# eniac/Reef

Hardware: AMD Instinct MI355X
Metric: msm_scalar_point_pairs_per_sec (higher is better)
Workload: dtype u32

## Files before the change

### reef_amd/csrc/api.cpp

```cpp
#include <stdarg.h>
#include <stdio.h>
#include <string>
#include <vector>
#include <new>
#include <exception>
#include <stdlib.h>
#include <string.h>

#include <atomic>
#include <chrono>
#include <condition_variable>
#include <deque>
#include <memory>
#include <mutex>
#include <thread>
#include <type_traits>

#include "common.h"
#include "keccak.h"

namespace reef {

static thread_local char g_err[512] = "";

// ... 1056 lines not shown
        j.copy = nullptr;
        g_cache_bytes -= j.key->charged; g_host_bytes -= j.key->host_charged;
        j.key->charged = j.key->host_charged = 0;
        int expect = 1;
        j.key->state.compare_exchange_strong(expect, state, std::memory_order_release);
    }
    void execute(Job &j) {
        if (j.kind == RETIRE) {
            ReadyCtx victim = give(j.device, j.retire);
            victim.destroy();
            return;
        }
        if (j.kind == PURGE) {
            std::vector<ReadyCtx> gone;
            {
                std::lock_guard<std::mutex> lk(mu);
                for (auto &v : spares)
                    for (size_t i = 0; i < v.size();)
                        if (v[i].key && v[i].key->state.load() == 3) { gone.push_back(v[i]); v.erase(v.begin() + i); }
                        else ++i;
            }
            for (auto &r : gone) r.destroy();
            return;
        }
        DeviceGuard dg(j.device);
        if (!dg.ok) { if (j.kind == BUILD) fail_build(j, 4); return; }
        SharedKey &k = *j.key;
        if (k.n >= BG_STREAM_MIN_POINTS) (void)stream_pool().ensure_background_stream(k.device);
        reef_msm_opts o = {};
        o.bucket_groups = 1;
        o.byte_tables = 2;
        o.device = k.device;
        reef_msm_ctx *master = nullptr;
        if (reef_msm_ctx_create(&master, k.curve, (const reef_affine *)j.copy, k.n, REEF_HOST, &o) != REEF_OK) { fail_build(j, 4); return; }
        k.host_copy = j.copy;
        k.master = master;
        j.copy = nullptr;
        ReadyCtx spare;
        if (ready_ctx_make(&spare, j.key, k.n) != REEF_OK) spare.destroy();
        g_cache_builds += 1;
        ReadyCtx old;
        if (spare.ctx) {
            old = give(k.curve, spare);
            g_cache_spares += 1;
            if (old.ctx == spare.ctx) { spare.destroy(); old = ReadyCtx(); }
        }
        int expect = 1;
        if (!k.state.compare_exchange_strong(expect, 2, std::memory_order_release) && spare.ctx) {
            bool mine = false;
            {
                std::lock_guard<std::mutex> lk(mu);
                auto &v = spares[k.curve];
                for (size_t i = 0; i < v.size(); ++i)
                    if (v[i].ctx == spare.ctx) { v.erase(v.begin() + i); mine = true; break; }
            }
            if (mine) spare.destroy();
        }
        if (old.ctx) old.destroy();
    }
};
Builder &Builder::builder_instance() {
    static Builder *b = new Builder();
    return *b;
}
static Builder &builder() { return Builder::builder_instance(); }

void KeyTable::clear() {
// ... 305 lines not shown
```

### reef_amd/csrc/common.h

```cpp
#pragma once
#include <algorithm>
#include <atomic>
#include <mutex>
#include <optional>
#include <thread>
#include <stdio.h>
#include <stdlib.h>
#include <vector>
#include <hip/hip_runtime.h>
#include <stddef.h>
#include <stdint.h>

#include "../../include/reef_msm.h"

namespace reef {

void set_error(const char *fmt, ...) __attribute__((format(printf, 1, 2)));

#define REEF_HIP_TRY(expr)                                                                          \
    do {                                                                                            \
        hipError_t e_ = (expr);                                                                     \
        if (e_ != hipSuccess) {                                                                     \
            ::reef::set_error("%s: %s (%s:%d)", #expr, hipGetErrorString(e_), __FILE__, __LINE__);  \
            return e_ == hipErrorOutOfMemory ? REEF_ERR_OOM : REEF_ERR_HIP;                         \
        }                                                                                           \
    } while (0)

#define REEF_TRY(expr)                          \
    do {                                        \
        reef_status s_ = (expr);                \
        if (s_ != REEF_OK) return s_;           \
    } while (0)

inline const char *exp_env(const char *name) {
#ifdef REEF_EXPERIMENT
    return getenv(name);
#else
    (void)name;
    return nullptr;
#endif
}

struct DeviceGuard {
    int prev = -1;
    bool switched = false, ok = true;
    hipError_t err = hipSuccess;
    explicit DeviceGuard(int dev) {
        err = hipGetDevice(&prev);
        if (err == hipSuccess && prev != dev) {
            err = hipSetDevice(dev);
            switched = err == hipSuccess;
        }
        ok = err == hipSuccess;
        if (!ok) (void)hipGetLastError();
    }
    ~DeviceGuard() {
        if (switched) (void)hipSetDevice(prev);
    }
    DeviceGuard(const DeviceGuard &) = delete;
    DeviceGuard &operator=(const DeviceGuard &) = delete;
};
#define REEF_ON_DEVICE(dev)                                                                                   \
    ::reef::DeviceGuard dg_((dev));                                                                           \
    if (!dg_.ok) {                                                                                            \
        ::reef::set_error("cannot make device %d current: %s", (int)(dev), hipGetErrorString(dg_.err));       \
        return REEF_ERR_HIP;                                                                                  \
    }

inline std::atomic<uint64_t> g_devbuf_gen{0};
struct DevBuf {
    void *p = nullptr;
    size_t cap = 0;
    reef_status ensure(size_t bytes) {
        if (bytes <= cap) return REEF_OK;
// ... 469 lines not shown
```

### reef_amd/csrc/ec.h

```cpp
#pragma once
#include "field.h"

#if defined(__HIP_DEVICE_COMPILE__)
#define REEF_ANY(x) __any(x)
#else
#define REEF_ANY(x) (x)
#endif

namespace reef {

struct affine {
    fe x, y;
};
struct xyzz {
    fe x, y, zz, zzz;
};
struct alignas(16) affine256 {
    fe256 x, y;
};
struct alignas(16) jacobian256 {
    fe256 x, y, z;
};
struct alignas(16) xyzz_mem {
    u32 w[36];
// ... 35 lines not shown

template <int C> REEF_HD xyzz xyzz_dbl_affine(const affine &p) {
    xyzz r;
    const fe u = fe_dbl<C>(p.y);
    const fe v = fe_sqr<C>(u);
    const fe w = fe_mul<C>(u, v);
    const fe s = fe_mul<C>(p.x, v);
    const fe xx = fe_sqr<C>(p.x);
    const fe m = fe_add<C>(fe_dbl<C>(xx), xx);
    r.x = fe_sub<C, 4>(fe_sqr<C>(m), fe_dbl<C>(s));
    r.y = fe_sub<C, 2>(fe_mul<C>(m, fe_sub<C, 8>(s, r.x)),
                       fe_mul<C>(w, p.y));
    r.zz = v;
    r.zzz = w;
    return r;
}

template <int C> REEF_HD xyzz xyzz_dbl(const xyzz &p) {
    xyzz r;
    const fe u = fe_dbl<C>(p.y);
    const fe v = fe_sqr<C>(u);
    const fe w = fe_mul<C>(u, v);
    const fe s = fe_mul<C>(p.x, v);
    const fe xx = fe_sqr<C>(p.x);
    const fe m = fe_add<C>(fe_dbl<C>(xx), xx);
    r.x = fe_sub<C, 4>(fe_sqr<C>(m), fe_dbl<C>(s));
    r.y = fe_sub<C, 2>(fe_mul<C>(m, fe_sub<C, 8>(s, r.x)),
                       fe_mul<C>(w, p.y));
    r.zz = fe_mul<C>(v, p.zz);
    r.zzz = fe_mul<C>(w, p.zzz);
    return r;
}

template <int C> REEF_HD xyzz xyzz_madd_flag(const xyzz &a, bool a_known_empty, const affine &p) {
    const bool a_inf = a_known_empty || xyzz_is_inf<C>(a);
    const bool p_inf = affine_is_inf(p);
    const fe pp_ = fe_mul_sub<C, 8>(p.x, a.zz, a.x);
    const fe rr = fe_mul_sub<C, 4>(p.y, a.zzz, a.y);
    xyzz r;
    if (__builtin_expect(fe_is_zero<C>(pp_) && fe_is_zero<C>(rr) && !a_inf && !p_inf, 0)) {
        r = xyzz_dbl_affine<C>(p);
    } else {
        const fe pp = fe_sqr<C>(pp_);
        const fe ppp = fe_mul<C>(pp_, pp);
        const fe q = fe_mul<C>(a.x, pp);
        fe t;
#pragma unroll
        for (int i = 0; i < 9; ++i) t.l[i] = ppp.l[i] + 2u * q.l[i];
        REEF_SET_BOUND(t, REEF_GET_BOUND(ppp) + 2.0 * REEF_GET_BOUND(q));
        r.x = fe_sqr_sub<C, 4>(rr, t);
        r.y = fe_mul2_add<C>(rr, fe_sub<C, 8>(q, r.x), fe_neg<C, 4>(a.y), ppp);
        r.zz = fe_mul<C>(a.zz, pp);
        r.zzz = fe_mul<C>(a.zzz, ppp);
    }
    if (REEF_ANY(a_inf)) {
        xyzz from_p;
        from_p.x = p.x; from_p.y = p.y; from_p.zz = fe_one<C>(); from_p.zzz = from_p.zz;
        r = xyzz_select(a_inf, from_p, r);
    }
    if (REEF_ANY(p_inf)) r = xyzz_select(p_inf, a, r);
    return r;
}

template <int C> REEF_HD xyzz xyzz_madd(const xyzz &a, const affine &p) { return xyzz_madd_flag<C>(a, false, p); }

template <int C> REEF_HD xyzz xyzz_add(const xyzz &a, const xyzz &b) {
    const bool a_inf = xyzz_is_inf<C>(a);
    const bool b_inf = xyzz_is_inf<C>(b);
    const fe u1 = fe_mul<C>(a.x, b.zz);
    const fe u2 = fe_mul<C>(b.x, a.zz);
    const fe s1 = fe_mul<C>(a.y, b.zzz);
    const fe s2 = fe_mul<C>(b.y, a.zzz);
    const fe pp_ = fe_sub<C, 2>(u2, u1);
    const fe rr = fe_sub<C, 2>(s2, s1);
    xyzz r;
    if (__builtin_expect(fe_is_zero<C>(pp_) && fe_is_zero<C>(rr) && !a_inf && !b_inf, 0)) {
        r = xyzz_dbl<C>(a);
    } else {
        const fe pp = fe_sqr<C>(pp_);
        const fe ppp = fe_mul<C>(pp_, pp);
        const fe q = fe_mul<C>(u1, pp);
        const fe t = fe_add<C>(ppp, fe_dbl<C>(q));
        r.x = fe_sub<C, 4>(fe_sqr<C>(rr), t);
        r.y = fe_mul2_add<C>(rr, fe_sub<C, 8>(q, r.x), fe_neg<C, 2>(s1), ppp);
        r.zz = fe_mul<C>(fe_mul<C>(a.zz, b.zz), pp);
        r.zzz = fe_mul<C>(fe_mul<C>(a.zzz, b.zzz), ppp);
    }
    r = xyzz_select(a_inf, b, r);
    r = xyzz_select(b_inf, a, r);
    return r;
}

REEF_HD affine affine_from_table(const affine256 &m) {
    affine r;
    r.x = fe_from_table(m.x);
    r.y = fe_from_table(m.y);
    return r;
}
template <int C> REEF_HD affine256 affine_to_table(const affine &p) {
    affine256 m;
    m.x = fe_to_table<C>(p.x);
    m.y = fe_to_table<C>(p.y);
    return m;
}
template <int C> REEF_HD affine affine_from_abi(const affine256 &m) {
    affine r;
    r.x = fe_from_abi<C>(m.x);
    r.y = fe_from_abi<C>(m.y);
    return r;
}
template <int C> REEF_HD affine256 affine_to_abi(const affine &p) {
    affine256 m;
    m.x = fe_to_abi<C>(p.x);
    m.y = fe_to_abi<C>(p.y);
    return m;
}
REEF_HD xyzz xyzz_from_mem(const xyzz_mem &m) {
    xyzz r;
#pragma unroll
    for (int i = 0; i < 9; ++i) {
        r.x.l[i] = m.w[i]; r.y.l[i] = m.w[9 + i]; r.zz.l[i] = m.w[18 + i]; r.zzz.l[i] = m.w[27 + i];
    }
    REEF_SET_BOUND(r.x, 6.0); REEF_SET_BOUND(r.y, 3.6); REEF_SET_BOUND(r.zz, 1.6); REEF_SET_BOUND(r.zzz, 1.6);
    return r;
}
REEF_HD xyzz_mem xyzz_to_mem(const xyzz &p) {
    xyzz_mem m;
#if defined(REEF_BOUNDS)
    if (p.x.bound > 6.0 || p.y.bound > 3.6 || p.zz.bound > 1.6 || p.zzz.bound > 1.6) REEF_BOUND_FAIL("xyzz_to_mem: invariant");
#endif
#pragma unroll
// ... 62 lines not shown
```

### reef_amd/csrc/engine.inc

```
#include <algorithm>
#include <atomic>
#include <mutex>
#include <string.h>
#include <vector>

#include "common.h"
#include "glv_host.h"
#include "host_combine.h"

namespace reef {

static_assert(sizeof(fe256) == sizeof(reef_fe), "fe256 layout");
static_assert(sizeof(affine256) == sizeof(reef_affine), "affine256 layout");
static_assert(sizeof(jacobian256) == sizeof(reef_jacobian), "jacobian256 layout");
static_assert(sizeof(xyzz_mem) == 144, "xyzz_mem layout");

static constexpr u32 MAX_LDS_KEYS = 32768;
static constexpr u32 MAX_SCAN_KEYS = SCAN_TILE * 1024;
static constexpr u32 SORT_SHIFT = 8;
static constexpr u64 TWO_LEVEL_MIN_ENTRIES = 1u << 20;
static constexpr u32 DEFAULT_L0 = 0;

static inline u32 ceil_div(u64 a, u64 b) { return (u32)((a + b - 1) / b); }
static inline u64 round_up(u64 a, u64 b) { return (a + b - 1) / b * b; }
static inline u32 windows_for(u32 c) { return (256 + c - 1) / c; }

static u32 choose_window(size_t n, u32 groups_mode ) {
    if (groups_mode == 1) {
        return n < 61440 ? 13u : n < 180224 ? 15u : 17u;
    }
    u32 best_c = 4;
    double best = 1e300;
    for (u32 c = 3; c <= 20; ++c) {
        const u32 W = windows_for(c);
        const u32 G = groups_mode == 0 ? W : std::min(groups_mode, W);
        const double nb = (double)(1u << (c - 1));
        const double digits = (double)(255 / c) + ((255 % c) == 0 ? 0.5 : 1.0);
        const double cost = digits * (double)n + (G == 1 ? 10.0 : 4.0) * G * nb;
        if (cost < best) { best = cost; best_c = c; }
    }
    return best_c;
}

template <int C> struct Key {
    affine256 *tables = nullptr;
    size_t n = 0, cap = 0;
    u32 c = 0, W = 0, G = 0, T = 0;
    affine256 *small_tab = nullptr;
    size_t small_n = 0;
    affine256 *wide_tab = nullptr;
    std::atomic<size_t> wide_n{0};
    std::atomic<int> wide_state{0};
    hipStream_t wide_stream = nullptr;
    hipEvent_t wide_event = nullptr;
    void *wide_stage = nullptr;
    int *wide_abort = nullptr;
    std::mutex wide_mu;
    std::atomic<int> refs{1};
    int device = 0;
};

template <int C> struct Ctx {
    Key<C> *key = nullptr;
    hipStream_t stream = nullptr;
    StreamLease lease;
    std::mutex mu;
    u32 opt_c = 0, opt_G = 0, L0 = DEFAULT_L0, opt_tables = 0;
    DevBuf scalars, blinds, hpoint, result, tmp_xyzz, maxbits;
    DevBuf dig, counts, tile_sums, bstart, entries;
    DevBuf bstart1, seg_first, seg_counts, entries1;
    DevBuf bucket_acc, lkeys[2], lvals[2];
    DevBuf rowcol, group_sums;
    static constexpr int EV_RING = 32;
    hipEvent_t evr[EV_RING][4] = {};
    bool ev_pending[EV_RING] = {};
    int ev_next = 0, ev_last = -1;
    hipEvent_t *ev = nullptr;
    double sum_total_ms = 0, sum_accum_ms = 0;
    u64 timed_calls = 0;
    jacobian256 *pinned = nullptr;
// ... 47 lines not shown
    REEF_HIP_TRY(hipEventSynchronize(ctx->evr[slot][3]));
    float t = 0, a = 0;
    REEF_HIP_TRY(hipEventElapsedTime(&t, ctx->evr[slot][0], ctx->evr[slot][3]));
    REEF_HIP_TRY(hipEventElapsedTime(&a, ctx->evr[slot][1], ctx->evr[slot][2]));
    ctx->sum_total_ms += t;
    ctx->sum_accum_ms += a;
    ctx->timed_calls += 1;
    ctx->ev_pending[slot] = false;
    return REEF_OK;
}
template <int C> static reef_status ctx_begin_timing(Ctx<C> *ctx) {
    const int slot = ctx->ev_next;
    REEF_TRY(ctx_harvest<C>(ctx, slot));
    ctx->ev = ctx->evr[slot];
    ctx->ev_last = slot;
    ctx->ev_next = (slot + 1) % Ctx<C>::EV_RING;
    return REEF_OK;
}

template <int C> static void wide_drop(Key<C> *k) {
    if (k->wide_abort) *(volatile int *)k->wide_abort = 1;
    if (k->wide_stream) (void)hipStreamSynchronize(k->wide_stream);
    if (k->wide_event) { (void)hipEventDestroy(k->wide_event); k->wide_event = nullptr; }
    if (k->wide_stream) { (void)hipStreamDestroy(k->wide_stream); k->wide_stream = nullptr; }
    if (k->wide_stage) { (void)hipFree(k->wide_stage); k->wide_stage = nullptr; }
    if (k->wide_tab) { (void)hipFree(k->wide_tab); k->wide_tab = nullptr; }
    if (k->wide_abort) { (void)hipHostFree(k->wide_abort); k->wide_abort = nullptr; }
    k->wide_n.store(0);
    k->wide_state.store(0);
}
template <int C> static void key_release(Key<C> *k) {
    if (k && --k->refs == 0) {
        if (k->tables) (void)hipFree(k->tables);
        if (k->small_tab) (void)hipFree(k->small_tab);
        wide_drop(k);
        delete k;
    }
}

static reef_status set_lds_limit(const void *fn) {
    REEF_HIP_TRY(hipFuncSetAttribute(fn, hipFuncAttributeMaxDynamicSharedMemorySize, (int)(MAX_LDS_KEYS * sizeof(u32))));
    return REEF_OK;
}

static reef_status engine_init_once() {
    static std::once_flag once;
    static reef_status st = REEF_OK;
    std::call_once(once, [] {
        auto f = []() -> reef_status {
            REEF_TRY(set_lds_limit((const void *)k_count));
            REEF_TRY(set_lds_limit((const void *)k_recode_count<REEF_CURVE>));
            REEF_TRY(set_lds_limit((const void *)k_scatter<false>));
            REEF_TRY(set_lds_limit((const void *)k_scatter<true>));
            REEF_TRY(set_lds_limit((const void *)k_row_count));
            REEF_TRY(set_lds_limit((const void *)k_row_scatter));
            return REEF_OK;
        };
        st = f();
    });
    return st;
}

static reef_status plan_for(size_t n, uint32_t c_opt, uint32_t g_opt, uint32_t *c, uint32_t *w, uint32_t *g, uint32_t *t);

static inline size_t small_table_points(size_t n) { return (size_t)SMALL_WINDOWS * SMALL_DIGITS * n; }
template <int C> static reef_status small_build(Ctx<C> *ctx, const affine256 *pts, size_t n, affine256 *out) {
// ... 167 lines not shown
    hipStream_t st = ctx->stream;
    const u64 total = (u64)WIDE_WINDOWS * n;
    const u32 per = wide_per(total);
    const u32 wgs = (u32)ceil_div(total, (u64)256 * per);
    REEF_TRY(ctx->wide_dig.ensure(total * sizeof(short)));
    const u32 lvl2 = ceil_div(wgs, 64);
    REEF_TRY(ctx->wide_partial.ensure(((size_t)wgs + lvl2) * sizeof(xyzz_mem)));
    xyzz_mem *p1 = ctx->wide_partial.template as<xyzz_mem>(), *p2 = p1 + wgs;
    if (ctx->timing) {
        REEF_TRY(ctx_begin_timing<C>(ctx));
        REEF_HIP_TRY(hipEventRecord(ctx->ev[0], st));
    }
    hipLaunchKernelGGL(k_wide_recode<C>, dim3(ceil_div(n, 256)), dim3(256), 0, st, d_scalars, (u32)n, (int)is_mont, ctx->wide_dig.template as<short>());
    if (ctx->timing) REEF_HIP_TRY(hipEventRecord(ctx->ev[1], st));
    hipLaunchKernelGGL((k_wide_accum<C, false>), dim3(wgs), dim3(256), 0, st, (const affine256 *)key->wide_tab, (u32)key->wide_n.load(),
                       (const short *)ctx->wide_dig.template as<short>(), (u32)n, per, 0u, p1);
    if (ctx->timing) REEF_HIP_TRY(hipEventRecord(ctx->ev[2], st));
    const xyzz_mem *last = p1;
    u32 cnt = wgs;
    if (cnt > 512) {
        hipLaunchKernelGGL(k_wide_reduce<C>, dim3(lvl2), dim3(256), 0, st, (const xyzz_mem *)p1, cnt, p2);
        last = p2;
        cnt = lvl2;
    }
    hipLaunchKernelGGL(k_small_final<C>, dim3(1), dim3(256), 0, st, last, cnt, d_out);
    if (ctx->timing) {
        REEF_HIP_TRY(hipEventRecord(ctx->ev[3], st));
        ctx->ev_pending[ctx->ev_last] = true;
    }
    REEF_HIP_TRY(hipGetLastError());
    return REEF_OK;
}

template <int C>
static reef_status key_build(Ctx<C> *ctx, const reef_affine *bases, size_t n, int loc) {
    Key<C> *key = ctx->key;
    u32 c, W, G, T;
    REEF_TRY(plan_for(n, ctx->opt_c, ctx->opt_G, &c, &W, &G, &T));
    wide_drop(key);
    const size_t need = (size_t)T * std::max<size_t>(n, 1);
    if (need > key->cap) {
        if (key->tables) { (void)hipFree(key->tables); key->tables = nullptr; key->cap = 0; }
        REEF_HIP_TRY(hipMalloc((void **)&key->tables, need * sizeof(affine256)));
        key->cap = need;
    }
    key->n = n; key->c = c; key->W = W; key->G = G; key->T = T;
    ctx->sym_bits = ctx->symw_bits = 0;
    graphs_clear(ctx);
    if (n == 0) return REEF_OK;
    const affine256 *src = (const affine256 *)bases;
    const u32 per_batch = T > 1 ? (u32)std::max<size_t>(1, std::min<size_t>(T - 1, (size_t(1) << 30) / (n * sizeof(xyzz_mem)))) : 1;
    size_t staging_bytes = T > 1 ? (size_t)per_batch * n * sizeof(xyzz_mem) : 0;
    if (G == 1 && n <= SMALL_N_MAX) staging_bytes = std::max(staging_bytes, (small_table_points(n) + (size_t)SMALL_WINDOWS * n) * sizeof(xyzz_mem));
    if (loc != REEF_DEVICE) staging_bytes = std::max(staging_bytes, n * sizeof(affine256));
    REEF_TRY(ctx->tmp_xyzz.ensure(std::max<size_t>(staging_bytes, 16)));
    if (loc != REEF_DEVICE) {
        REEF_HIP_TRY(hipMemcpyAsync(ctx->tmp_xyzz.p, bases, n * sizeof(affine256), hipMemcpyHostToDevice, ctx->stream));
        src = ctx->tmp_xyzz.template as<affine256>();
    }
    hipLaunchKernelGGL(k_import_key<C>, dim3(ceil_div(n, 256)), dim3(256), 0, ctx->stream, src, (u32)n, key->tables);
    if (T > 1) {
        for (u32 j = 1; j < T; j += per_batch) {
            const u32 cnt = std::min(per_batch, T - j);
            hipLaunchKernelGGL(k_shift_chain<C>, dim3(ceil_div(n, 64)), dim3(64), 0, ctx->stream, key->tables + (size_t)(j - 1) * n, (u32)n, c * G, cnt, 0,
                               ctx->tmp_xyzz.template as<xyzz_mem>());
            hipLaunchKernelGGL((k_xyzz_normalize<C, false>), dim3(ceil_div(ceil_div((size_t)cnt * n, NORM_PER), 256)), dim3(256), 0, ctx->stream,
                               ctx->tmp_xyzz.template as<xyzz_mem>(), (u32)((size_t)cnt * n), key->tables + (size_t)j * n);
        }
    }
    key->small_n = 0;
    if (G == 1 && n <= SMALL_N_MAX) {
        if (key->small_tab) { (void)hipFree(key->small_tab); key->small_tab = nullptr; }
        REEF_HIP_TRY(hipMalloc((void **)&key->small_tab, small_table_points(n) * sizeof(affine256)));
        REEF_TRY(small_build<C>(ctx, key->tables, n, key->small_tab));
        key->small_n = n;
    }
    REEF_HIP_TRY(hipGetLastError());
    REEF_HIP_TRY(hipStreamSynchronize(ctx->stream));
    if (ctx->tmp_xyzz.cap > (size_t(96) << 20)) ctx->tmp_xyzz.release();
    if (wide_start<C>(key, ctx->opt_tables) != REEF_OK) {
        (void)hipGetLastError();
        wide_drop(key);
    }
    if (ctx->opt_tables == 1) wide_poll<C>(key, true);
    return REEF_OK;
}

template <int C> static void ctx_free(Ctx<C> *ctx) {
    if (!ctx) return;
    ctx_free(ctx->side);
    ctx_free(ctx->side_batch);
    for (auto &e : ctx->batch_ev)
        if (e) (void)hipEventDestroy(e);
    graphs_clear(ctx);
    for (DevBuf *b : {&ctx->scalars, &ctx->blinds, &ctx->hpoint, &ctx->dig, &ctx->counts, &ctx->bstart, &ctx->bstart1, &ctx->seg_first,
                      &ctx->seg_counts, &ctx->entries1, &ctx->sym_table, &ctx->sym_tmp, &ctx->sym_u8, &ctx->tile_sums,
                      &ctx->entries, &ctx->bucket_acc, &ctx->rowcol, &ctx->group_sums, &ctx->result,
                      &ctx->tmp_xyzz, &ctx->maxbits, &ctx->wsum, &ctx->deep_dig, &ctx->deep_part, &ctx->h_tab, &ctx->small_partial, &ctx->wide_dig, &ctx->wide_partial, &ctx->lkeys[0], &ctx->lkeys[1], &ctx->lvals[0], &ctx->lvals[1]})
        b->release();
    for (auto &q : ctx->evr)
        for (auto &e : q)
            if (e) (void)hipEventDestroy(e);
// ... 389 lines not shown
            hipLaunchKernelGGL(k_seg_plan, dim3(1), dim3(1024), 0, st, bstart_c, NBTc, seg_first);
            hipLaunchKernelGGL(k_fine_count<true>, dim3(nseg_max), dim3(1024), fine * sizeof(u32), st, (const void *)e1, bstart_c, seg_first, NBTc, shift, seg_counts);
            hipLaunchKernelGGL(k_fine_offsets, dim3(NBTc), dim3(fine), 0, st, bstart_c, seg_first, NBTc, shift, seg_counts, bstart);
            if (word_entries)
                hipLaunchKernelGGL((k_fine_scatter<true, true>), dim3(nseg_max), dim3(1024), fine * sizeof(u32), st, (const void *)e1, bstart_c, seg_first, NBTc, shift, seg_counts,
                                   (void *)ctx->entries.template as<u32x2>());
            else
                hipLaunchKernelGGL((k_fine_scatter<true, false>), dim3(nseg_max), dim3(1024), fine * sizeof(u32), st, (const void *)e1, bstart_c, seg_first, NBTc, shift, seg_counts,
                                   (void *)ctx->entries.template as<u32x2>());
        } else {
            hipLaunchKernelGGL(k_scatter<false>, dim3(S, groups_total, NBc / sh.KB), dim3(1024), sh.KB * sizeof(u32), st, dig, sh, ctx->counts.template as<u32>(), (void *)e1);
            hipLaunchKernelGGL(k_seg_plan, dim3(1), dim3(1024), 0, st, bstart_c, NBTc, seg_first);
            hipLaunchKernelGGL(k_fine_count<false>, dim3(nseg_max), dim3(1024), fine * sizeof(u32), st, (const void *)e1, bstart_c, seg_first, NBTc, shift, seg_counts);
            hipLaunchKernelGGL(k_fine_offsets, dim3(NBTc), dim3(fine), 0, st, bstart_c, seg_first, NBTc, shift, seg_counts, bstart);
            hipLaunchKernelGGL((k_fine_scatter<false, false>), dim3(nseg_max), dim3(1024), fine * sizeof(u32), st, (const void *)e1, bstart_c, seg_first, NBTc, shift, seg_counts,
                               (void *)ctx->entries.template as<u32x2>());
        }
    } else if (!row_mode) {
        hipLaunchKernelGGL(k_scatter<false>, dim3(S, groups_total, NB / sh.KB), dim3(1024), sh.KB * sizeof(u32), st, dig, sh, ctx->counts.template as<u32>(),
                           (void *)ctx->entries.template as<u32x2>());
    } else {
        hipLaunchKernelGGL(k_row_scatter, dim3(ceil_div(pl.rows, rsh.rows_per_block)), dim3(1024),
                           rsh.rows_per_block * pl.G * NB * sizeof(u32), st, dig, rsh, bstart, ctx->entries.template as<u32x2>());
    }

    if (ctx->timing) REEF_HIP_TRY(hipEventRecord(ctx->ev[1], st));
    const bool fused = merge_is_fused<C>(ctx, nchunks0);
    {
        const dim3 ag(ceil_div(nchunks0, 256)), ab(256);
        const void *ent = (const void *)ctx->entries.template as<u32x2>();
        xyzz_mem *bacc = ctx->bucket_acc.template as<xyzz_mem>();
        u32 *ok = ctx->lkeys[fused ? 1 : 0].template as<u32>();
        xyzz_mem *ov = ctx->lvals[fused ? 1 : 0].template as<xyzz_mem>();
        if (fused && word_entries) hipLaunchKernelGGL((k_accum0<C, true, true>), ag, ab, 0, st, ctx->key->tables, ent, bstart + NBT, L0, nchunks0, bacc, ok, ov, NBT);
        else if (fused) hipLaunchKernelGGL((k_accum0<C, true, false>), ag, ab, 0, st, ctx->key->tables, ent, bstart + NBT, L0, nchunks0, bacc, ok, ov, 0u);
        else if (word_entries) hipLaunchKernelGGL((k_accum0<C, false, true>), ag, ab, 0, st, ctx->key->tables, ent, bstart + NBT, L0, nchunks0, bacc, ok, ov, NBT);
        else hipLaunchKernelGGL((k_accum0<C, false, false>), ag, ab, 0, st, ctx->key->tables, ent, bstart + NBT, L0, nchunks0, bacc, ok, ov, 0u);
    }
    if (ctx->timing) REEF_HIP_TRY(hipEventRecord(ctx->ev[2], st));
    launch_partial_merge<C>(ctx, nchunks0, ctx->bucket_acc.template as<xyzz_mem>(), fused);

    const u32 lg = pl.c - 1;
    const u32 c2 = (lg + 1) / 2, c1 = lg - c2;
    const u32 per_group = (1u << c1) + (1u << c2);
    const u32 rc_waves = groups_total * per_group;
    xyzz_mem *gsum = ctx->group_sums.template as<xyzz_mem>();
    if (group_sums_out && ctx->pinned && (size_t)groups_total * sizeof(xyzz_mem) <= Ctx<C>::PINNED_POINTS * sizeof(jacobian256))
        gsum = (xyzz_mem *)ctx->pinned;
    const bool direct = !group_sums_out && pl.G == 1;
    static const int skip_reduce = [] { const char *e = exp_env("REEF_MSM_SKIP_REDUCE"); return e ? atoi(e) : 0; }();
    const int lanes = rowcol >= 0 ? rowcol : rowcol_lanes<C>(ctx, NB);
    auto launch_rowcol = [&](auto lps) {
        constexpr int LPS = decltype(lps)::value;
        hipLaunchKernelGGL((k_reduce_rowcol<C, LPS>), dim3(ceil_div(ceil_div(rc_waves, 64u / LPS), 4)), dim3(256), 0, st, ctx->bucket_acc.template as<xyzz_mem>(),
                           bstart, c1, c2, groups_total, ctx->rowcol.template as<xyzz_mem>());
    };
    if (skip_reduce == 1) {
        if (group_sums_out) *group_sums_out = gsum;
    } else if (ctx->coop) {
        REEF_TRY(ctx->wsum.ensure((u64)groups_total * 4 * sizeof(xyzz_mem)));
        ++ctx->rowcol_calls[lanes != 0];
        if (skip_reduce == 2) {}
        else if (lanes == 16) launch_rowcol(std::integral_constant<int, 16>{});
        else if (lanes == 32) launch_rowcol(std::integral_constant<int, 32>{});
        else if (lanes == 64) launch_rowcol(std::integral_constant<int, 64>{});
        else
        hipLaunchKernelGGL(k_reduce_rowcol_coop<C>, dim3(rc_waves), dim3(256), 0, st, ctx->bucket_acc.template as<xyzz_mem>(), bstart, c1, c2,
                           groups_total, ctx->rowcol.template as<xyzz_mem>());
        hipLaunchKernelGGL(k_reduce_weighted_coop<C>, dim3(groups_total, 2), dim3(256), 0, st, ctx->rowcol.template as<xyzz_mem>(), c1, c2,
                           ctx->wsum.template as<xyzz_mem>());
// ... 1201 lines not shown
```

### reef_amd/csrc/msm_kernels.inc

```
#include "ec.h"
#include "ec_coop.h"
#include "glv_consts.h"

namespace reef {

static constexpr u32 KEY_INVALID = 0xffffffffu;
static constexpr int WAVE = 64;

template <int C> struct Kern;

__device__ __forceinline__ void latency_critical() { __builtin_amdgcn_s_setprio(3); }

__device__ __forceinline__ u32 extract_bits(const fe256 &k, u32 off, u32 c) {
    const u32 limb = off >> 5, sh = off & 31u;
    u32 lo = 0, hi = 0;
#pragma unroll
    for (u32 l = 0; l < 8; ++l) {
        lo = (l == limb) ? k.w[l] : lo;
        hi = (l == limb + 1) ? k.w[l] : hi;
    }
    u64 v = (((u64)hi << 32) | lo) >> sh;
    return (u32)v & ((1u << c) - 1u);
}

__device__ __forceinline__ fe256 load_fe256(const fe256 *p) {
    const u32x4 *q = reinterpret_cast<const u32x4 *>(p);
    const u32x4 a = q[0], b = q[1];
    fe256 d;
    d.w[0] = a.x; d.w[1] = a.y; d.w[2] = a.z; d.w[3] = a.w;
    d.w[4] = b.x; d.w[5] = b.y; d.w[6] = b.z; d.w[7] = b.w;
    return d;
}
__device__ __forceinline__ void store_fe256(fe256 *p, const fe256 &s) {
    u32x4 *q = reinterpret_cast<u32x4 *>(p);
    q[0] = mk_u32x4(s.w[0], s.w[1], s.w[2], s.w[3]);
    q[1] = mk_u32x4(s.w[4], s.w[5], s.w[6], s.w[7]);
}
__device__ __forceinline__ affine256 load_affine256(const affine256 *p) {
    affine256 r;
    r.x = load_fe256(&p->x);
    r.y = load_fe256(&p->y);
    return r;
}
__device__ __forceinline__ void store_affine256(affine256 *p, const affine256 &s) {
    store_fe256(&p->x, s.x);
    store_fe256(&p->y, s.y);
}
__device__ __forceinline__ jacobian256 load_jacobian256(const jacobian256 *p) {
    jacobian256 r;
    r.x = load_fe256(&p->x); r.y = load_fe256(&p->y); r.z = load_fe256(&p->z);
    return r;
}
__device__ __forceinline__ void store_jacobian256(jacobian256 *p, const jacobian256 &s) {
    store_fe256(&p->x, s.x); store_fe256(&p->y, s.y); store_fe256(&p->z, s.z);
}
__device__ __forceinline__ affine load_table_point(const affine256 *p) { return affine_from_table(load_affine256(p)); }
__device__ __forceinline__ xyzz load_xyzz(const xyzz_mem *p) {
    const u32x4 *q = reinterpret_cast<const u32x4 *>(p);
    xyzz_mem m;
#pragma unroll
    for (int i = 0; i < 9; ++i) {
        const u32x4 v = q[i];
        m.w[4 * i] = v.x; m.w[4 * i + 1] = v.y; m.w[4 * i + 2] = v.z; m.w[4 * i + 3] = v.w;
    }
    return xyzz_from_mem(m);
}
__device__ __forceinline__ xyzz load_xyzz_coop(const xyzz_mem *p) {
    const u32x4 *q = reinterpret_cast<const u32x4 *>(p);
    xyzz_mem m;
#pragma unroll
    for (int i = 0; i < 9; ++i) {
        const u32x4 v = q[i];
        m.w[4 * i] = coop_launder(v.x); m.w[4 * i + 1] = coop_launder(v.y); m.w[4 * i + 2] = coop_launder(v.z); m.w[4 * i + 3] = coop_launder(v.w);
    }
    return xyzz_from_mem(m);
}
__device__ __forceinline__ void store_xyzz(xyzz_mem *p, const xyzz &s) {
    const xyzz_mem m = xyzz_to_mem(s);
    u32x4 *q = reinterpret_cast<u32x4 *>(p);
#pragma unroll
    for (int i = 0; i < 9; ++i) q[i] = mk_u32x4(m.w[4 * i], m.w[4 * i + 1], m.w[4 * i + 2], m.w[4 * i + 3]);
}
__device__ __forceinline__ xyzz shfl_xyzz(const xyzz &a, int src_lane) {
    xyzz_mem m = xyzz_to_mem(a);
#pragma unroll
    for (int i = 0; i < 36; ++i) m.w[i] = __shfl(m.w[i], src_lane, WAVE);
    return xyzz_from_mem(m);
}

// ... 447 lines not shown
    for (u32 k = threadIdx.x; k < nkeys; k += blockDim.x) cur[k] = bucket_start[key0 + k];
    __syncthreads();
    const size_t n = (size_t)sh.rows * sh.row_len;
    const u32 cnt = nrows * sh.row_len;
    for (u32 w = 0; w < sh.W; ++w) {
        const u32 *d = dig + (size_t)w * n + (size_t)r0 * sh.row_len;
        const u32 g = w % sh.G, j = w / sh.G;
        for (u32 e = threadIdx.x; e < cnt; e += blockDim.x) {
            const u32 v = d[e];
            const u32 mag = v & 0x7fffffffu;
            if (mag) {
                const u32 row = e / sh.row_len, col = e - row * sh.row_len;
                const u32 rel = (row * sh.G + g) * sh.NB + mag - 1u;
                const u32 pos = atomicAdd(&cur[rel], 1u);
                entries[pos] = mk_u32x2(key0 + rel, (j * sh.n_ctx + col) | (v & 0x80000000u));
            }
        }
    }
}

template <int C, bool COOP>
__device__ __forceinline__ void merge_wave(u32 ka, u32 kb, xyzz v, xyzz bv, u32 wave_id, int lane, int role, CoopLds *L,
                                           xyzz_mem *__restrict__ bucket_acc, u32 *__restrict__ out_keys, xyzz_mem *__restrict__ out_vals);


__device__ __forceinline__ u32 bucket_of(const u32 *__restrict__ bs, u32 nbt, u32 p) {
    u32 lo = 0, hi = nbt;
    while (hi - lo > 1) {
        const u32 mid = (lo + hi) >> 1;
        if (bs[mid] <= p) lo = mid; else hi = mid;
    }
    return lo;
}
template <int C, bool FUSED, bool WORD = false>
__global__ void __launch_bounds__(256) k_accum0(const affine256 *__restrict__ tables, const void *__restrict__ entries_,
                                               const u32 *__restrict__ m_ptr, u32 L0,
                                               u32 nchunks, xyzz_mem *__restrict__ bucket_acc, u32 *__restrict__ out_keys,
                                               xyzz_mem *__restrict__ out_vals, u32 nbt = 0) {
    __shared__ xyzz_mem stash[FUSED ? 256 : 1];
    const u32 t = blockIdx.x * blockDim.x + threadIdx.x;
    if constexpr (FUSED) {
        if (((t >> 6) << 6) >= nchunks) return;
    } else {
        if (t >= nchunks) return;
    }
    const u32 M = *m_ptr;
    while (L0 > 8 && (u64)(L0 >> 1) * nchunks >= M) L0 >>= 1;
    const u32 start = t * L0;
    u32 key_a = KEY_INVALID, key_b = KEY_INVALID;
    xyzz tail = xyzz_identity();
    if (t < nchunks && start < M) {
        const u32 end = min(start + L0, M);
        const u32 cnt = end - start;
        const u32x2 *mine = static_cast<const u32x2 *>(entries_) + start;
        const u32 *mine1 = static_cast<const u32 *>(entries_) + start;
        const u32 *bs = m_ptr - nbt;
        u32 cur_key, pay, boundary = 0;
        bool lo_open, ro_open = false;
        u32 prev_key = KEY_INVALID, next_key = KEY_INVALID;
        if constexpr (WORD) {
            cur_key = bucket_of(bs, nbt, start);
            boundary = bs[cur_key + 1];
            lo_open = bs[cur_key] < start;
            pay = mine1[0];
        } else {
            prev_key = start > 0 ? static_cast<const u32x2 *>(entries_)[start - 1].x : KEY_INVALID;
            next_key = end < M ? static_cast<const u32x2 *>(entries_)[end].x : KEY_INVALID;
            const u32x2 e0 = mine[0];
            cur_key = e0.x;
            pay = e0.y;
            lo_open = prev_key == cur_key;
        }
        affine256 raw = load_affine256(tables + (pay & 0x7fffffffu));
        xyzz acc = xyzz_identity();
        bool acc_empty = true;
        bool first_run = true;
        for (u32 k = 0; k < cnt; ++k) {
            u32 nkey = cur_key, npay = 0;
            affine256 nraw = raw;
            if (k + 1 < cnt) {
                if constexpr (WORD) {
                    npay = mine1[k + 1];
                    if (start + k + 1 == boundary) {
                        nkey = cur_key + 1;
                        if (bs[nkey + 1] == boundary) nkey = bucket_of(bs, nbt, boundary);
                    }
                } else {
                    const u32x2 e = mine[k + 1];
                    nkey = e.x;
                    npay = e.y;
                }
                nraw = load_affine256(tables + (npay & 0x7fffffffu));
            }
            affine pt = affine_from_table(raw);
            pt.y = fe_select((pay >> 31) != 0 && !affine_is_inf(pt), fe_neg<C, 2>(pt.y), pt.y);
            acc = xyzz_madd_flag<C>(acc, acc_empty, pt);
            acc_empty = false;
            const bool last = (k + 1 == cnt);
            if (last || nkey != cur_key) {
                const bool lo = first_run && lo_open;
                bool ro;
                if constexpr (WORD) ro = last && boundary > end;
                else ro = last && next_key == cur_key;
                if (!lo && !ro) {
                    store_xyzz(bucket_acc + cur_key, acc);
                } else if (lo) {
                    if constexpr (FUSED) store_xyzz(&stash[threadIdx.x], acc);
                    else store_xyzz(out_vals + 2 * (size_t)t, acc);
                    key_a = cur_key;
                    if (ro) {
                        if constexpr (!FUSED) store_xyzz(out_vals + 2 * (size_t)t + 1, xyzz_identity());
                        key_b = cur_key;
                    }
                } else {
                    if constexpr (FUSED) tail = acc;
                    else store_xyzz(out_vals + 2 * (size_t)t + 1, acc);
                    key_b = cur_key;
                }
                first_run = false;
                acc = xyzz_identity();
                acc_empty = true;
                if constexpr (WORD) { if (!last) boundary = bs[nkey + 1]; }
            }
            cur_key = nkey; pay = npay; raw = nraw;
        }
        (void)ro_open; (void)prev_key;
    }
    if constexpr (FUSED) {
        latency_critical();
// ... 904 lines not shown
    __shared__ BatchInvShared inv_sh;
    const u32 t = blockIdx.x * blockDim.x + threadIdx.x;
    const u64 i0 = (u64)t * NORM_PER;
    fe zp[NORM_PER], pre[NORM_PER];
    fe acc = fe_one<C>();
#pragma unroll
    for (int k = 0; k < NORM_PER; ++k) {
        zp[k] = fe_one<C>();
        if (i0 + k < n) {
            const xyzz p = load_xyzz(in + i0 + k);
            const fe prod = fe_mul<C>(p.zz, p.zzz);
            zp[k] = fe_select(fe_is_zero<C>(prod), zp[k], prod);
        }
        pre[k] = acc;
        acc = fe_mul<C>(acc, zp[k]);
    }
    fe inv = block_batch_inverse<C>(acc, inv_sh);
#pragma unroll
    for (int k = NORM_PER - 1; k >= 0; --k) {
        const fe ti = fe_mul<C>(inv, pre[k]);
        inv = fe_mul<C>(inv, zp[k]);
        if (i0 + k < n) {
            const affine a = xyzz_to_affine_with_inv<C>(load_xyzz(in + i0 + k), ti);
            store_affine256(out + i0 + k, ABI_OUT ? affine_to_abi<C>(a) : affine_to_table<C>(a));
        }
    }
}

template <int C>
__global__ void __launch_bounds__(256) k_import_key(const affine256 *__restrict__ src, u32 n, affine256 *__restrict__ dst) {
    const u32 i = blockIdx.x * blockDim.x + threadIdx.x;
    if (i >= n) return;
    store_affine256(dst + i, affine_to_table<C>(affine_from_abi<C>(load_affine256(src + i))));
}

template <int C>
__global__ void __launch_bounds__(64) k_shift_chain(const affine256 *__restrict__ src, u32 n, u32 shift, u32 count, int first,
                                                    xyzz_mem *__restrict__ tmp) {
    const u32 i = blockIdx.x * blockDim.x + threadIdx.x;
    if (i >= n) return;
    xyzz p = xyzz_from_affine<C>(load_table_point(src + i));
    for (u32 j = 0; j < count; ++j) {
        if (!(first && j == 0))
            for (u32 s = 0; s < shift; ++s) p = xyzz_dbl<C>(p);
        store_xyzz(tmp + (size_t)j * n + i, p);
    }
}


template <int C>
__global__ void __launch_bounds__(256) k_sym_multiples(const affine256 *__restrict__ gens, u32 n, u32 lb, u32 hb, xyzz_mem *__restrict__ lo_out,
                                                      xyzz_mem *__restrict__ hi_out) {
    const u32 t = blockIdx.x * blockDim.x + threadIdx.x;
    const u32 j = t >> 1, part = t & 1u;
    if (j >= n || (part == 1 && hb == 0)) return;
    const affine g = load_table_point(gens + j);
    const u32 count = 1u << (part ? hb : lb);
    xyzz_mem *out = (part ? hi_out : lo_out) + (size_t)j * count;
    xyzz step = xyzz_from_affine<C>(g);
    if (part)
        for (u32 s = 0; s < lb; ++s) step = xyzz_dbl<C>(step);
    xyzz acc = xyzz_identity();
    store_xyzz(out, acc);
    for (u32 v = 1; v < count; ++v) {
        acc = part ? xyzz_add<C>(acc, step) : xyzz_madd<C>(acc, g);
        store_xyzz(out + v, acc);
// ... 574 lines not shown
```

Baseline: 910.7 million.

## Add precomputed limb tables with stored negated y for bucket accumulation

Builds a second per-key table in which each point is kept in unpacked limb form together with a precomputed negated y and an infinity flag. The accumulation kernel then loads x plus whichever y it needs, skipping the unpack, the negation and the infinity test in the inner loop. The next-entry prefetch is also made unconditional by clamping the index. The cost is extra device memory and a one-time conversion kernel per key. The cache-build path turns the feature off through a thread-local flag so that master contexts keep only the packed tables.

Measured after the change: 931.5 million (median of 6 runs). +2.3%, better.

```diff
diff --git a/reef_amd/csrc/api.cpp b/reef_amd/csrc/api.cpp
--- a/reef_amd/csrc/api.cpp
+++ b/reef_amd/csrc/api.cpp
@@ -1112,7 +1112,10 @@
         o.byte_tables = 2;
         o.device = k.device;
         reef_msm_ctx *master = nullptr;
-        if (reef_msm_ctx_create(&master, k.curve, (const reef_affine *)j.copy, k.n, REEF_HOST, &o) != REEF_OK) { fail_build(j, 4); return; }
+        tl_packed_tables_only = true;
+        const reef_status built = reef_msm_ctx_create(&master, k.curve, (const reef_affine *)j.copy, k.n, REEF_HOST, &o);
+        tl_packed_tables_only = false;
+        if (built != REEF_OK) { fail_build(j, 4); return; }
         k.host_copy = j.copy;
         k.master = master;
         j.copy = nullptr;
diff --git a/reef_amd/csrc/common.h b/reef_amd/csrc/common.h
--- a/reef_amd/csrc/common.h
+++ b/reef_amd/csrc/common.h
@@ -40,6 +40,8 @@
     return nullptr;
 #endif
 }
+
+inline thread_local bool tl_packed_tables_only = false;
 
 struct DeviceGuard {
     int prev = -1;
diff --git a/reef_amd/csrc/ec.h b/reef_amd/csrc/ec.h
--- a/reef_amd/csrc/ec.h
+++ b/reef_amd/csrc/ec.h
@@ -91,9 +91,8 @@
     return r;
 }
 
-template <int C> REEF_HD xyzz xyzz_madd_flag(const xyzz &a, bool a_known_empty, const affine &p) {
+template <int C> REEF_HD xyzz xyzz_madd_flags(const xyzz &a, bool a_known_empty, const affine &p, bool p_inf) {
     const bool a_inf = a_known_empty || xyzz_is_inf<C>(a);
-    const bool p_inf = affine_is_inf(p);
     const fe pp_ = fe_mul_sub<C, 8>(p.x, a.zz, a.x);
     const fe rr = fe_mul_sub<C, 4>(p.y, a.zzz, a.y);
     xyzz r;
@@ -119,6 +118,10 @@
     }
     if (REEF_ANY(p_inf)) r = xyzz_select(p_inf, a, r);
     return r;
+}
+
+template <int C> REEF_HD xyzz xyzz_madd_flag(const xyzz &a, bool a_known_empty, const affine &p) {
+    return xyzz_madd_flags<C>(a, a_known_empty, p, affine_is_inf(p));
 }
 
 template <int C> REEF_HD xyzz xyzz_madd(const xyzz &a, const affine &p) { return xyzz_madd_flag<C>(a, false, p); }
@@ -156,6 +159,40 @@
     r.y = fe_from_table(m.y);
     return r;
 }
+struct alignas(16) affine_limbs {
+    u32 w[32];
+};
+static constexpr int LIMBS_X = 0, LIMBS_TOP = 8, LIMBS_Y = 12, LIMBS_NEG_Y = 20;
+template <int C> REEF_HD affine_limbs affine_limbs_from_table(const affine256 &m) {
+    const affine p = affine_from_table(m);
+    const bool inf = affine_is_inf(p);
+    const fe ny = fe_select(inf, fe_zero(), fe_neg<C, 2>(p.y));
+    affine_limbs r;
+#pragma unroll
+    for (int i = 0; i < 8; ++i) {
+        r.w[LIMBS_X + i] = p.x.l[i];
+        r.w[LIMBS_Y + i] = p.y.l[i];
+        r.w[LIMBS_NEG_Y + i] = ny.l[i];
+    }
+    r.w[LIMBS_TOP] = p.x.l[8]; r.w[LIMBS_TOP + 1] = p.y.l[8]; r.w[LIMBS_TOP + 2] = ny.l[8]; r.w[LIMBS_TOP + 3] = inf ? 1u : 0u;
+#pragma unroll
+    for (int i = 28; i < 32; ++i) r.w[i] = 0;
+    return r;
+}
+struct limbs_entry {
+    u32 head[12], ysel[8];
+};
+REEF_HD affine affine_from_limbs(const limbs_entry &e, bool neg, bool *inf) {
+    affine r;
+#pragma unroll
+    for (int i = 0; i < 8; ++i) { r.x.l[i] = e.head[i]; r.y.l[i] = e.ysel[i]; }
+    r.x.l[8] = e.head[8];
+    r.y.l[8] = neg ? e.head[10] : e.head[9];
+    REEF_SET_BOUND(r.x, 1.0);
+    REEF_SET_BOUND(r.y, neg ? 2.0 : 1.0);
+    *inf = e.head[11] != 0;
+    return r;
+}
 template <int C> REEF_HD affine256 affine_to_table(const affine &p) {
     affine256 m;
     m.x = fe_to_table<C>(p.x);
diff --git a/reef_amd/csrc/engine.inc b/reef_amd/csrc/engine.inc
--- a/reef_amd/csrc/engine.inc
+++ b/reef_amd/csrc/engine.inc
@@ -46,6 +46,8 @@
     affine256 *tables = nullptr;
     size_t n = 0, cap = 0;
     u32 c = 0, W = 0, G = 0, T = 0;
+    affine_limbs *limb_tables = nullptr;
+    size_t limb_cap = 0;
     affine256 *small_tab = nullptr;
     size_t small_n = 0;
     affine256 *wide_tab = nullptr;
@@ -159,6 +161,7 @@
 template <int C> static void key_release(Key<C> *k) {
     if (k && --k->refs == 0) {
         if (k->tables) (void)hipFree(k->tables);
+        if (k->limb_tables) (void)hipFree(k->limb_tables);
         if (k->small_tab) (void)hipFree(k->small_tab);
         wide_drop(k);
         delete k;
@@ -392,6 +395,12 @@
     return REEF_OK;
 }
 
+static inline bool limb_tables_wanted(size_t n, u32 G, u32 T, u32 opt_tables) {
+    if (n == 0 || T <= 1 || (u64)T * n >= (1ull << 31) || tl_packed_tables_only) return false;
+    if (G == 1 && (n <= SMALL_N_MAX || (wide_enabled(opt_tables) && n <= wide_n_max()))) return false;
+    const char *e = exp_env("REEF_MSM_LIMB_TABLES");
+    return !(e && atoi(e) == 0);
+}
 template <int C>
 static reef_status key_build(Ctx<C> *ctx, const reef_affine *bases, size_t n, int loc) {
     Key<C> *key = ctx->key;
@@ -407,6 +416,12 @@
     key->n = n; key->c = c; key->W = W; key->G = G; key->T = T;
     ctx->sym_bits = ctx->symw_bits = 0;
     graphs_clear(ctx);
+    const bool limbs = limb_tables_wanted(n, G, T, ctx->opt_tables);
+    if (key->limb_tables && (!limbs || need > key->limb_cap)) { (void)hipFree(key->limb_tables); key->limb_tables = nullptr; key->limb_cap = 0; }
+    if (limbs && !key->limb_tables) {
+        if (hipMalloc((void **)&key->limb_tables, need * sizeof(affine_limbs)) == hipSuccess) key->limb_cap = need;
+        else { (void)hipGetLastError(); key->limb_tables = nullptr; }
+    }
     if (n == 0) return REEF_OK;
     const affine256 *src = (const affine256 *)bases;
     const u32 per_batch = T > 1 ? (u32)std::max<size_t>(1, std::min<size_t>(T - 1, (size_t(1) << 30) / (n * sizeof(xyzz_mem)))) : 1;
@@ -428,6 +443,9 @@
                                ctx->tmp_xyzz.template as<xyzz_mem>(), (u32)((size_t)cnt * n), key->tables + (size_t)j * n);
         }
     }
+    if (key->limb_tables)
+        hipLaunchKernelGGL(k_limb_tables<C>, dim3(ceil_div((size_t)T * n, 256)), dim3(256), 0, ctx->stream, (const affine256 *)key->tables, (u32)((size_t)T * n),
+                           key->limb_tables);
     key->small_n = 0;
     if (G == 1 && n <= SMALL_N_MAX) {
         if (key->small_tab) { (void)hipFree(key->small_tab); key->small_tab = nullptr; }
@@ -883,10 +901,15 @@
         xyzz_mem *bacc = ctx->bucket_acc.template as<xyzz_mem>();
         u32 *ok = ctx->lkeys[fused ? 1 : 0].template as<u32>();
         xyzz_mem *ov = ctx->lvals[fused ? 1 : 0].template as<xyzz_mem>();
-        if (fused && word_entries) hipLaunchKernelGGL((k_accum0<C, true, true>), ag, ab, 0, st, ctx->key->tables, ent, bstart + NBT, L0, nchunks0, bacc, ok, ov, NBT);
-        else if (fused) hipLaunchKernelGGL((k_accum0<C, true, false>), ag, ab, 0, st, ctx->key->tables, ent, bstart + NBT, L0, nchunks0, bacc, ok, ov, 0u);
-        else if (word_entries) hipLaunchKernelGGL((k_accum0<C, false, true>), ag, ab, 0, st, ctx->key->tables, ent, bstart + NBT, L0, nchunks0, bacc, ok, ov, NBT);
-        else hipLaunchKernelGGL((k_accum0<C, false, false>), ag, ab, 0, st, ctx->key->tables, ent, bstart + NBT, L0, nchunks0, bacc, ok, ov, 0u);
+        auto launch_accum0 = [&](const auto *tables) {
+            using TABLE = std::remove_cv_t<std::remove_pointer_t<decltype(tables)>>;
+            if (fused && word_entries) hipLaunchKernelGGL((k_accum0<C, true, true, TABLE>), ag, ab, 0, st, tables, ent, bstart + NBT, L0, nchunks0, bacc, ok, ov, NBT);
+            else if (fused) hipLaunchKernelGGL((k_accum0<C, true, false, TABLE>), ag, ab, 0, st, tables, ent, bstart + NBT, L0, nchunks0, bacc, ok, ov, 0u);
+            else if (word_entries) hipLaunchKernelGGL((k_accum0<C, false, true, TABLE>), ag, ab, 0, st, tables, ent, bstart + NBT, L0, nchunks0, bacc, ok, ov, NBT);
+            else hipLaunchKernelGGL((k_accum0<C, false, false, TABLE>), ag, ab, 0, st, tables, ent, bstart + NBT, L0, nchunks0, bacc, ok, ov, 0u);
+        };
+        if (ctx->key->limb_tables) launch_accum0((const affine_limbs *)ctx->key->limb_tables);
+        else launch_accum0((const affine256 *)ctx->key->tables);
     }
     if (ctx->timing) REEF_HIP_TRY(hipEventRecord(ctx->ev[2], st));
     launch_partial_merge<C>(ctx, nchunks0, ctx->bucket_acc.template as<xyzz_mem>(), fused);
diff --git a/reef_amd/csrc/msm_kernels.inc b/reef_amd/csrc/msm_kernels.inc
--- a/reef_amd/csrc/msm_kernels.inc
+++ b/reef_amd/csrc/msm_kernels.inc
@@ -1,3 +1,5 @@
+#include <type_traits>
+
 #include "ec.h"
 #include "ec_coop.h"
 #include "glv_consts.h"
@@ -55,6 +57,22 @@
     store_fe256(&p->x, s.x); store_fe256(&p->y, s.y); store_fe256(&p->z, s.z);
 }
 __device__ __forceinline__ affine load_table_point(const affine256 *p) { return affine_from_table(load_affine256(p)); }
+__device__ __forceinline__ limbs_entry load_limbs_entry(const affine_limbs *p, bool neg) {
+    const u32x4 *q = reinterpret_cast<const u32x4 *>(p);
+    const u32x4 *qy = q + (neg ? LIMBS_NEG_Y / 4 : LIMBS_Y / 4);
+    const u32x4 a = q[0], b = q[1], c = q[2], d = qy[0], e = qy[1];
+    limbs_entry r;
+    r.head[0] = a.x; r.head[1] = a.y; r.head[2] = a.z; r.head[3] = a.w;
+    r.head[4] = b.x; r.head[5] = b.y; r.head[6] = b.z; r.head[7] = b.w;
+    r.head[8] = c.x; r.head[9] = c.y; r.head[10] = c.z; r.head[11] = c.w;
+    r.ysel[0] = d.x; r.ysel[1] = d.y; r.ysel[2] = d.z; r.ysel[3] = d.w;
+    r.ysel[4] = e.x; r.ysel[5] = e.y; r.ysel[6] = e.z; r.ysel[7] = e.w;
+    return r;
+}
+__device__ __forceinline__ affine256 load_accum_entry(const affine256 *tables, u32 pay) { return load_affine256(tables + (pay & 0x7fffffffu)); }
+__device__ __forceinline__ limbs_entry load_accum_entry(const affine_limbs *tables, u32 pay) {
+    return load_limbs_entry(tables + (pay & 0x7fffffffu), (pay >> 31) != 0);
+}
 __device__ __forceinline__ xyzz load_xyzz(const xyzz_mem *p) {
     const u32x4 *q = reinterpret_cast<const u32x4 *>(p);
     xyzz_mem m;
@@ -568,8 +586,8 @@
     }
     return lo;
 }
-template <int C, bool FUSED, bool WORD = false>
-__global__ void __launch_bounds__(256) k_accum0(const affine256 *__restrict__ tables, const void *__restrict__ entries_,
+template <int C, bool FUSED, bool WORD = false, typename TABLE = affine256>
+__global__ void __launch_bounds__(256) k_accum0(const TABLE *__restrict__ tables, const void *__restrict__ entries_,
                                                const u32 *__restrict__ m_ptr, u32 L0,
                                                u32 nchunks, xyzz_mem *__restrict__ bucket_acc, u32 *__restrict__ out_keys,
                                                xyzz_mem *__restrict__ out_vals, u32 nbt = 0) {
@@ -607,30 +625,34 @@
             pay = e0.y;
             lo_open = prev_key == cur_key;
         }
-        affine256 raw = load_affine256(tables + (pay & 0x7fffffffu));
+        auto raw = load_accum_entry(tables, pay);
         xyzz acc = xyzz_identity();
         bool acc_empty = true;
         bool first_run = true;
         for (u32 k = 0; k < cnt; ++k) {
-            u32 nkey = cur_key, npay = 0;
-            affine256 nraw = raw;
-            if (k + 1 < cnt) {
-                if constexpr (WORD) {
-                    npay = mine1[k + 1];
-                    if (start + k + 1 == boundary) {
-                        nkey = cur_key + 1;
-                        if (bs[nkey + 1] == boundary) nkey = bucket_of(bs, nbt, boundary);
-                    }
-                } else {
-                    const u32x2 e = mine[k + 1];
-                    nkey = e.x;
-                    npay = e.y;
+            const u32 kn = k + 1 < cnt ? k + 1 : k;
+            u32 nkey = cur_key, npay;
+            if constexpr (WORD) {
+                npay = mine1[kn];
+                if (k + 1 < cnt && start + k + 1 == boundary) {
+                    nkey = cur_key + 1;
+                    if (bs[nkey + 1] == boundary) nkey = bucket_of(bs, nbt, boundary);
                 }
-                nraw = load_affine256(tables + (npay & 0x7fffffffu));
+            } else {
+                const u32x2 e = mine[kn];
+                nkey = e.x;
+                npay = e.y;
             }
-            affine pt = affine_from_table(raw);
-            pt.y = fe_select((pay >> 31) != 0 && !affine_is_inf(pt), fe_neg<C, 2>(pt.y), pt.y);
-            acc = xyzz_madd_flag<C>(acc, acc_empty, pt);
+            const auto nraw = load_accum_entry(tables, npay);
+            if constexpr (std::is_same<TABLE, affine_limbs>::value) {
+                bool pt_inf;
+                const affine pt = affine_from_limbs(raw, (pay >> 31) != 0, &pt_inf);
+                acc = xyzz_madd_flags<C>(acc, acc_empty, pt, pt_inf);
+            } else {
+                affine pt = affine_from_table(raw);
+                pt.y = fe_select((pay >> 31) != 0 && !affine_is_inf(pt), fe_neg<C, 2>(pt.y), pt.y);
+                acc = xyzz_madd_flag<C>(acc, acc_empty, pt);
+            }
             acc_empty = false;
             const bool last = (k + 1 == cnt);
             if (last || nkey != cur_key) {
@@ -1601,6 +1623,16 @@
     const u32 i = blockIdx.x * blockDim.x + threadIdx.x;
     if (i >= n) return;
     store_affine256(dst + i, affine_to_table<C>(affine_from_abi<C>(load_affine256(src + i))));
+}
+
+template <int C>
+__global__ void __launch_bounds__(256) k_limb_tables(const affine256 *__restrict__ src, u32 count, affine_limbs *__restrict__ dst) {
+    const u32 i = blockIdx.x * blockDim.x + threadIdx.x;
+    if (i >= count) return;
+    const affine_limbs r = affine_limbs_from_table<C>(load_affine256(src + i));
+    u32x4 *q = reinterpret_cast<u32x4 *>(dst + i);
+#pragma unroll
+    for (int k = 0; k < 8; ++k) q[k] = mk_u32x4(r.w[4 * k], r.w[4 * k + 1], r.w[4 * k + 2], r.w[4 * k + 3]);
 }
 
 template <int C>
```
